# alasdairforsythe/tokenmonster

Measured on AMD Instinct MI355X. Metric: GB/s raw UTF-8 tokenized, englishcode-32000 vocab, higher is better.
Workload: dtype u8; 1 GPU; englishcode-32000-consistent vocabulary shape (synthetic, 32000 ids / 54181 index records), 1024 MiB raw synthetic mixed text per GPU in 300327 documents; end to end: input = RAW UTF-8 resident in HBM, normalized (NFD+capcode) on the GPU inside the timed step, output = uint32 ids + offsets in HBM; raw_bytes_per_gpu=1073743404, normalized_bytes_per_gpu=1145560274, missing=0, parallelism=documents sharded by rank, no collective, rccl_ranks=0

## Files before the change

### tokenmonster_amd/csrc/tm_kernels.hip

```cpp
#include <hip/hip_runtime.h>

#include <algorithm>
#include <chrono>
#include <cstring>
#include <type_traits>
#include <vector>

#include "tm_pipeline.h"

namespace tmh {


__global__ void k_doc_nseg(const uint64_t* __restrict__ doc_begin, const uint64_t* __restrict__ doc_end, uint32_t ndocs,
                           uint32_t* __restrict__ doc_nseg, uint32_t unit = SEG, uint32_t* __restrict__ zero_word = nullptr) {
  uint32_t d = blockIdx.x * blockDim.x + threadIdx.x;
  if (zero_word && d == 0) *zero_word = 0u;
  if (d < ndocs) {
    uint64_t len = doc_end[d] - doc_begin[d];
    doc_nseg[d] = (uint32_t)((len + unit - 1) / unit);
  }
}


__global__ void k_scan_partial(const uint32_t* __restrict__ in, uint64_t n, uint64_t* __restrict__ block_sums) {
// ... 152 lines not shown

template <int FD>
__device__ __forceinline__ uint32_t transition(const Tables& T, const WaveLds& w, const uint8_t* s_bb, int p, int dl,
                                               uint32_t d, const Row& O) {
  if (d == 0) return (T.unk_id != TM_NONE ? T.unk_id : ID_NONE) | (1u << 24) | (1u << 31);
  const int len = (int)desc_len(d);
  const uint32_t id = O.x & kRowIdMask;
  const int i1 = p + len;
  uint32_t res = id | ((uint32_t)len << 24);
  if (i1 < dl && ((O.w & (1u << 21)) == 0 || ((d >> D_NEXT_SPACE) & 1u) == 0u)) {
    const int len1 = (int)(O.w & 63u), len2 = (int)((O.w >> 6) & 63u);
    const int flen[3] = {len, len1 - FD, len2 - FD};
    const int fpart[3] = {len + (int)(O.x >> kRowIdBits) - FD * (100 + (int)((O.w >> 18) & 1u)),
                          (int)(O.y >> kRowIdBits) - FD * (101 + (int)((O.w >> 19) & 1u)),
                          (int)(O.z >> kRowIdBits) - FD * (101 + (int)((O.w >> 20) & 1u))};
    const uint32_t fb[3] = {((O.w >> 12) & 1u) | (((O.w >> 15) & 1u) << 8), ((O.w >> 13) & 1u) | (((O.w >> 16) & 1u) << 8),
                            ((O.w >> 14) & 1u) | (((O.w >> 17) & 1u) << 8)};
    const int nk = len1 == 0 ? 1 : (len2 == 0 ? 2 : 3);
    int best = NOSCORE, bestb = NOSCORE;
    uint32_t resb = 0;
#pragma unroll
    for (int k = 0; k < 3; k++) {
      if (k < nk) {
        const int ik = p + flen[k];
        const uint32_t dS = w.D[ik];
        if (dS != 0) {
          int sc = branch_score(fpart[k], fb[k], dS, false);
          if (k > 0) sc -= alt_penalty(flen[k], dS, len);
          const uint32_t rk = (k == 0 ? id : ((k == 1 ? O.y : O.z) & kRowIdMask)) | ((uint32_t)flen[k] << 24);
          if (sc > best) { best = sc; res = rk; }
          if (dS & D_HAS_B) {
            const uint32_t dB = w.Db[ik];
            int sb = branch_score(fpart[k], fb[k], dB, true);
            if (k > 0) sb -= alt_penalty(flen[k], dB, len);
            if (sb > bestb) { bestb = sb; resb = rk | (1u << 30); }
          }
        }
      }
    }
    if (bestb > best) res = resb;
  }
  return res;
}

#if defined(TM_DEVEL) || defined(TM_PHASE_TIMERS)
#include "../../tools/devel/tm_devel.h"
#else
#define TM_DBG_ON(x) false
#define PH_INIT
#define PH_INC(i)
#define PH_FLUSH
#define PH(i)
#define PH_COUNT(i, n)
#endif


constexpr uint32_t SP_DL_BITS = 21, SP_LEN_SHIFT = 21, SP_LEN_BITS = 9, SP_SAME_DOC = 1u << 30, SP_MORE_TEXT = 1u << 31, SP_DL_MAX = 1u << 20;
static_assert(SP_DL_MAX < (1u << SP_DL_BITS) && SEG < (1 << SP_LEN_BITS) && SP_LEN_SHIFT + SP_LEN_BITS == 30, "the packed word of a segment record");
__global__ void k_seg_fill(const uint64_t* __restrict__ doc_seg_start, uint32_t ndocs, const uint64_t* __restrict__ doc_begin, const uint64_t* __restrict__ doc_end,
                           const uint64_t* __restrict__ doc_vis, const uint64_t* __restrict__ doc_piece_start, const uint64_t* __restrict__ piece_off, uint64_t nseg,
                           uint32_t* __restrict__ seg_doc, uint4* __restrict__ seg_src, const uint64_t* __restrict__ ctl = nullptr) {
  const uint64_t g = (uint64_t)blockIdx.x * blockDim.x + threadIdx.x;
  if (ctl) nseg = ctl[0];
  if (g >= nseg) return;
  uint32_t dl = 0, dh = ndocs;
  while (dh - dl > 1) {
    const uint32_t mid = dl + (dh - dl) / 2;
    if (doc_seg_start[mid] <= g) dl = mid; else dh = mid;
  }
  seg_doc[g] = dl;
  const uint64_t begin = doc_begin[dl] + (g - doc_seg_start[dl]) * SEG;
  const uint64_t rem = doc_end[dl] - begin, remv = doc_vis[dl] - begin;
  const uint32_t look = remv > (uint64_t)SP_DL_MAX ? SP_DL_MAX : (uint32_t)remv;
  const uint32_t seglen = rem < (uint64_t)SEG ? (uint32_t)rem : (uint32_t)SEG;
  const bool same = g + 1 < nseg && doc_seg_start[dl + 1] > g + 1;
  const uint32_t w = look | (seglen << SP_LEN_SHIFT) | (same ? SP_SAME_DOC : 0u) | (remv > (uint64_t)seglen ? SP_MORE_TEXT : 0u);
  if (doc_piece_start == nullptr) { seg_src[g] = make_uint4((uint32_t)begin, (uint32_t)(begin >> 32) & 0xFFu, 0u, w); return; }
  uint64_t lo = doc_piece_start[dl], hi = doc_piece_start[dl + 1];
  while (hi - lo > 1) {
    const uint64_t mid = (lo + hi) >> 1;
    if (piece_off[mid] <= begin) lo = mid; else hi = mid;
  }
  seg_src[g] = make_uint4((uint32_t)lo, (uint32_t)(begin - piece_off[lo]), (uint32_t)(piece_off[lo + 1] - begin), w);
}

constexpr int J_SKIP = NPOS - SEG, J_PLANE = NPOS;
constexpr int TAIL_TASK0 = 64, TAIL_TASKS = (NPOS - TAIL_TASK0) / 3, REDO0 = 160, REDO_WORDS = (NPOS + 31) / 32;
static_assert(REDO0 + REDO_WORDS <= SEG && offsetof(WaveLds, Db) + 4 * 63 + 6 * 256 + 4 <= offsetof(WaveLds, Xb) + 4 * REDO0, "the bitmap lies behind the dump words");
__global__ __launch_bounds__(WAVES * 64, 8) void k_match_branch(Tables T, const uint8_t* __restrict__ text, uint64_t nseg,
                                                                uint32_t* __restrict__ R0, uint2* __restrict__ side,
                                                                uint32_t* __restrict__ R1, uint32_t* __restrict__ exitmap, uint16_t* __restrict__ exit16,
                                                                int narrow, int dbg, const uint8_t* __restrict__ slab, const uint4* __restrict__ par,
                                                                const uint64_t* __restrict__ ctl = nullptr) {
  __shared__ uint8_t s_bb[256];
  __shared__ WaveLds s_wave[WAVES];
  const int lane = threadIdx.x & 63, wvi = __builtin_amdgcn_readfirstlane((int)(threadIdx.x >> 6));
  TM_LDS_OBJECTS(s_bb, s_wave);
  PH_INIT
  const uint64_t g = (uint64_t)blockIdx.x * WAVES + wvi;
  const uint8_t* const bbp = T.begin_byte;
  const uint4 rec = par[g < nseg ? g : nseg - 1];
  if (ctl) nseg = ctl[0];
  TM_HAVE_IN_SGPRS6(rec.x, rec.w, nseg, text, slab, bbp);
  const uint32_t bbw = reinterpret_cast<const uint32_t*>(bbp)[lane];
  if (g >= nseg) return;
  WaveLds& w = s_wave[wvi];
// ... 434 lines not shown
#pragma unroll
    for (int k = 0; k < N0; k++)
      if (pend(ja[k]) && (ja[k] >> JF) >= (uint32_t)SEG) ja[k] = (ja[k] & JCNT) + J1[(ja[k] >> JF) - SEG];
    for (int round = 0; round < 6; round++) {
      bool anyb = false;
#pragma unroll
      for (int k = 0; k < N0; k++) anyb |= pend(ja[k]) && (ja[k] >> (JF + 6)) == (uint32_t)k;
      if (__builtin_amdgcn_ballot_w64(anyb) == 0ull) break;
#pragma unroll
      for (int k = 0; k < N0; k++) {
        const uint32_t b = bperm(ja[k], ja[k]);
        ja[k] = pend(ja[k]) && (ja[k] >> (JF + 6)) == (uint32_t)k ? (ja[k] & JCNT) + b : ja[k];
      }
      PH_INC(13)
    }
#pragma unroll
    for (int k = N0 - 2; k >= 0; k--) {
      uint32_t b = 0u;
#pragma unroll
      for (int j = k + 1; j < N0; j++) {
        const uint32_t bj = bperm(ja[k], ja[j]);
        b = (ja[k] >> (JF + 6)) == (uint32_t)j ? bj : b;
      }
      ja[k] = pend(ja[k]) ? (ja[k] & JCNT) + b : ja[k];
    }
    uint32_t e1 = jb[0];
    if (__builtin_amdgcn_ballot_w64(lane < ENT / 2 && pend(e1)) != 0ull) {
      uint32_t b = 0u;
#pragma unroll
      for (int j = 0; j < N0; j++) {
        const uint32_t bj = bperm(e1, ja[j]);
        b = (e1 >> (JF + 6)) == (uint32_t)j ? bj : b;
      }
      e1 = pend(e1) ? (e1 & JCNT) + b : e1;
    }
    const bool all_wide = (dbg & 32) != 0;
    auto ok_of = [](uint32_t a) { return (a >> 31) != 0 && ((a >> JF) & JNONE) != JNONE; };
    auto e16 = [&](uint32_t a) -> uint32_t { return ok_of(a) ? (((a >> JF) & JNONE) | ((all_wide ? 511u : min(a & JCNT, 511u)) << 7)) : 0xFFFFu; };
    if (lane < ENT / 2) *reinterpret_cast<uint32_t*>(exit16 + g * ENT + 2 * lane) = e16(ja[0]) | (e16(e1) << 16);
    const bool wide = all_wide || (lane < ENT / 2 && ((ok_of(ja[0]) && (ja[0] & JCNT) >= 511u) || (ok_of(e1) && (e1 & JCNT) >= 511u)));
    if (__any(wide) && lane < ENT / 2) {
      exitmap[g * ENT + 2 * lane] = ok_of(ja[0]) ? ((ja[0] >> JF) & JNONE) | ((ja[0] & JCNT) << 8) : R_INVALID;
      exitmap[g * ENT + 2 * lane + 1] = ok_of(e1) ? ((e1 >> JF) & JNONE) | ((e1 & JCNT) << 8) : R_INVALID;
    }
  }
  PH(7)
  PH_FLUSH
}


__global__ void k_resolve(const uint32_t* __restrict__ exitmap, const uint16_t* __restrict__ exit16, const uint64_t* __restrict__ doc_seg_start, uint32_t ndocs,
                          const uint8_t* __restrict__ doc_entry, uint8_t* __restrict__ seg_entry, uint32_t* __restrict__ seg_tokbase,
                          uint32_t* __restrict__ doc_ntok, uint32_t* __restrict__ error_flag, uint32_t long_segs, uint32_t* __restrict__ doc_fd,
                          uint32_t* __restrict__ doc_missing, const uint64_t* __restrict__ ctl = nullptr) {
  uint32_t d = blockIdx.x * blockDim.x + threadIdx.x;
  if (ctl && d < ndocs && ctl[1] == 0) { doc_ntok[d] = 0u; return; }
  if (d >= ndocs) return;
  doc_fd[d] = 0u; doc_missing[d] = 0u;
  uint64_t g0 = doc_seg_start[d], g1 = doc_seg_start[d + 1];
  if (g1 - g0 > long_segs) return;
  uint32_t e = doc_entry ? doc_entry[d] : 0u, ntok = 0;
  for (uint64_t g = g0; g < g1; g++) {
    seg_entry[g] = (uint8_t)e;
    seg_tokbase[g] = ntok;
    const uint32_t x = exit_entry(exit16, exitmap, g * ENT + e);
    if (x == R_INVALID) { atomicOr(error_flag, 1u); break; }
    e = x & 0xFFu;
    ntok += x >> 8;
  }
  doc_ntok[d] = ntok;
}


template <bool LEAF>
__global__ __launch_bounds__(128) void k_group_compose(const uint32_t* __restrict__ exitmap, const uint16_t* __restrict__ exit16, const uint2* __restrict__ gmap_in, const Group* __restrict__ groups,
                                                       uint32_t first_group, uint2* __restrict__ gmap) {
  const uint32_t gi = first_group + blockIdx.x;
  const Group gr = groups[gi];
  const uint32_t e0 = threadIdx.x;
  if (e0 >= ENT) return;
  uint32_t e = e0, ntok = 0;
  bool ok = true;
  for (uint32_t k = 0; k < gr.nchildren; k++) {
    if (LEAF) {
      const uint32_t x = exit_entry(exit16, exitmap, (uint64_t)(gr.first_child + k) * ENT + e);
      if (x == R_INVALID) { ok = false; break; }
      e = x & 0xFFu;
      ntok += x >> 8;
    } else {
      const uint2 x = gmap_in[(uint64_t)(gr.first_child + k) * ENT + e];
      if (x.x == R_INVALID) { ok = false; break; }
      e = x.x;
      ntok += x.y;
    }
  }
  gmap[(uint64_t)gi * ENT + e0] = ok ? make_uint2(e, ntok) : make_uint2(R_INVALID, 0u);
}

__global__ void k_long_top(const uint2* __restrict__ gmap, const LongDoc* __restrict__ longs, uint32_t nlong, const uint8_t* __restrict__ doc_entry,
                           uint8_t* __restrict__ group_entry, uint32_t* __restrict__ group_base, uint32_t* __restrict__ doc_ntok,
                           uint32_t* __restrict__ error_flag) {
  const uint32_t i = blockIdx.x * blockDim.x + threadIdx.x;
  if (i >= nlong) return;
  const LongDoc ld = longs[i];
  uint32_t e = doc_entry ? doc_entry[ld.doc] : 0u, ntok = 0;
  for (uint32_t k = 0; k < ld.ngroups; k++) {
    const uint32_t gi = ld.first_group + k;
    group_entry[gi] = (uint8_t)e;
    group_base[gi] = ntok;
    const uint2 x = gmap[(uint64_t)gi * ENT + e];
    if (x.x == R_INVALID) { atomicOr(error_flag, 1u); break; }
    e = x.x;
    ntok += x.y;
  }
  doc_ntok[ld.doc] = ntok;
}

template <bool LEAF>
__global__ void k_group_expand(const uint32_t* __restrict__ exitmap, const uint16_t* __restrict__ exit16, const uint2* __restrict__ gmap, const Group* __restrict__ groups, uint32_t first_group,
                               uint32_t ngroups, uint8_t* __restrict__ group_entry, uint32_t* __restrict__ group_base,
                               uint8_t* __restrict__ seg_entry, uint32_t* __restrict__ seg_tokbase, uint32_t* __restrict__ error_flag) {
  const uint32_t t = blockIdx.x * blockDim.x + threadIdx.x;
  if (t >= ngroups) return;
// ... 349 lines not shown
            nmiss += w >> 31;
            if (fits) {
              if (NARROW) { if (id != ID_NONE) rowa[E++] = (uint16_t)id; if (fd) rowa[E++] = (uint16_t)delete_id; }
              else { if (id != ID_NONE) row[E++] = id; if (fd) row[E++] = delete_id; }
            } else {
              if (id != ID_NONE) { if (t.base + E < out_cap) TM_STREAM_STORE(&out[t.base + E], id); E++; }
              if (fd) { if (t.base + E < out_cap) TM_STREAM_STORE(&out[t.base + E], delete_id); E++; }
            }
            p += (w >> 24) & 63u;
            hop++;
            gate = p < seglen ? slack0 + (int)p - (int)E - (int)((fd | direct) << 16) : GATE_DEAD;
          }
        }
      } else if (__builtin_amdgcn_ballot_w64(gate >= 0) == 0ull) break;
    }
    if (direct == 0u) staged = E;
    if (nfd | nmiss) {
      const uint32_t doc = seg_doc[g0 + lane];
      if (nfd) atomicAdd(&doc_fd[doc], nfd);
      if (nmiss) atomicAdd(&doc_missing[doc], nmiss);
    }
  }
  __builtin_amdgcn_wave_barrier();
  __builtin_amdgcn_s_waitcnt(0);
#pragma unroll 4
  for (int s = 0; s < nv; s++) {
    const uint32_t n = (uint32_t)__shfl((int)staged, s);
    const uint64_t base = shfl_u64(t.base, s);
    for (uint32_t j = (uint32_t)lane; j < n; j += 64u) if (base + j < out_cap) TM_STREAM_STORE(&out[base + j], NARROW ? (uint32_t)s_a[NARROW ? s : 0][j] : s_tile[NARROW ? 0 : s][j]);
  }
}

template <bool WIDE, bool OUT16 = false>
__global__ __launch_bounds__(64) void k_emit_list(const uint32_t* __restrict__ R0, const uint2* __restrict__ side,
                                                  const uint32_t* __restrict__ R1, const uint4* __restrict__ par, uint64_t nseg,
                                                  uint32_t delete_id, uint64_t out_cap, uint32_t* __restrict__ out,
                                                  uint32_t* __restrict__ error_flag, uint32_t stage_after, const uint32_t* __restrict__ seg_doc,
                                                  uint32_t* __restrict__ doc_fd, uint32_t* __restrict__ doc_missing, uint32_t no_id,
                                                  const uint64_t* __restrict__ ctl = nullptr) {
  alignas(16) __shared__ uint8_t s_m[TSL][TROW_L];
  __shared__ uint32_t s_side[TSL][9];
  __shared__ uint32_t s_n[TSL];
  __shared__ uint64_t s_base[TSL];
  const int lane = threadIdx.x;
  const uint64_t g0 = (uint64_t)blockIdx.x * TSL;
  if (ctl) { nseg = ctl[0]; if (g0 >= nseg) return; }
  const int nv = (int)(nseg - g0 < (uint64_t)TSL ? nseg - g0 : (uint64_t)TSL);
  const TileSeg t = tile_segment(par, g0 + lane, lane < TSL, nseg);
  constexpr uint32_t SLACK = TSLACK_L;
  const uint8_t* rows_g = reinterpret_cast<const uint8_t*>(R0);
  typedef typename std::conditional<WIDE, uint32_t, uint16_t>::type idt;
  typedef typename std::conditional<OUT16, uint16_t, uint32_t>::type outt;
  outt* const outp = reinterpret_cast<outt*>(out);
  constexpr uint64_t RS = WIDE ? R0_WIDE : R0_NARROW, FO = WIDE ? 4 * SEG : 2 * SEG;
  {
    uint32_t vb[TSL];
#pragma unroll
    for (int s = 0; s < TSL; s++) {
      const int ss = s < nv ? s : nv - 1;
      const uint32_t len = s < nv ? (uint32_t)__shfl((int)t.seglen, ss) : 0u;
      vb[s] = 0u;
      if (4u * (uint32_t)lane < len) vb[s] = TM_STREAM_LOAD(reinterpret_cast<const uint32_t*>(rows_g + (g0 + (uint64_t)ss) * RS + FO) + lane);
    }
#pragma unroll
    for (int s = 0; s < TSL; s++) *reinterpret_cast<uint32_t*>(&s_m[s][TSLACK_L + 4 * lane]) = vb[s];
#pragma unroll
    for (int i = lane; i < TSL * 9; i += 64) reinterpret_cast<uint32_t*>(s_side)[i] = 0u;
    static_assert((TSL & (TSL - 1)) == 0 && TSL >= 8 && TSL <= 64, "a lane per segment, lane & (TSL - 1); the second phase takes eight at a time");
    __builtin_amdgcn_wave_barrier();
    __builtin_amdgcn_s_waitcnt(0);
  }
  uint32_t staged = 0;
  {
    const int rl = lane & (TSL - 1);
    uint8_t* rowm = s_m[rl];
    uint32_t* smap = s_side[rl];
    const uint2* __restrict__ sl = side + (g0 + rl) * SIDE_STRIDE;
    const idt* __restrict__ ids_g = reinterpret_cast<const idt*>(rows_g + (g0 + (uint64_t)(rl < nv ? rl : 0)) * RS);
    uint32_t nfd = 0, nmiss = 0;
    auto word = [&](uint32_t pp, uint32_t f) -> uint32_t {
      if (f != 0) return side_word(sl, R1, g0 + rl, pp);
      const uint32_t m8 = rowm[SLACK + pp];
      return ((m8 >> 7) ? no_id : (uint32_t)ids_g[pp]) | ((m8 & 63u) << 24) | ((m8 >> 6) << 30);
    };
    const uint32_t seglen = t.have ? t.seglen : 0u;
    uint32_t p = t.entry >> 1, fd = t.entry & 1u, E = 0, direct = 0, hop = 0;
    constexpr int GATE_DEAD = -(1 << 24);
    const int slack0 = (int)SLACK - 2 - (int)stage_after;
    int gate = p < seglen ? slack0 + (int)p - (int)(fd << 16) : GATE_DEAD;
    const uint32_t nounk = no_id == ID_NONE ? 1u : 0u;
    auto fast_step = [&]() __attribute__((always_inline)) {
      const uint32_t m8 = rowm[SLACK + p];
      const uint32_t miss = m8 >> 7, fdn = (m8 >> 6) & 1u, adv = m8 & 63u;
      const uint32_t has = 1u - (miss & nounk);
      rowm[E] = (uint8_t)p; E += has; rowm[E] = (uint8_t)p;
      E += fdn;
      gate += (int)adv - (int)(fdn * 0x10001u + has);
      nfd += fdn;
      nmiss += miss;
      fd = fdn;
      p += max(adv, 1u);
      gate = p < seglen ? gate : GATE_DEAD;
    };
    for (;;) {
#ifndef TM_EMU
      if (gate >= 0) {
        do fast_step(); while (__builtin_amdgcn_ballot_w64(gate < 0) == 0ull);
      }
#else
      if (__builtin_amdgcn_ballot_w64(gate >= 0) != 0ull) {
        const bool in = gate >= 0;
        do { if (in) fast_step(); } while (__builtin_amdgcn_ballot_w64(in && gate < 0) == 0ull);
      }
#endif
      const bool general = (uint32_t)gate > (uint32_t)GATE_DEAD;
      if (__builtin_amdgcn_ballot_w64(general) != 0ull) {
        if (general) {
          const uint32_t w = word(p, fd);
          if (w == R_INVALID || hop > 2u * SEG) { atomicOr(error_flag, 2u); p = seglen; gate = GATE_DEAD; }
          else {
            const uint32_t id = w & ID_NONE, adv = (w >> 24) & 63u, fdn = (w >> 30) & 1u;
            const bool fits = direct == 0u && slack0 + (int)p - (int)E >= 0 && adv != 0u && !(id == ID_NONE && fdn != 0u);
            if (!fits && direct == 0u) { direct = 1u; staged = E; }
            nfd += fdn;
            nmiss += w >> 31;
            if (fits) {
              if (id != ID_NONE) {
                if (fd) { smap[E >> 5] |= 1u << (E & 31u); if (t.base + E < out_cap) TM_STREAM_STORE(&outp[t.base + E], (outt)id); }
                rowm[E++] = (uint8_t)p;
              }
              if (fdn) rowm[E++] = (uint8_t)p;
            } else {
              if (id != ID_NONE) { if (t.base + E < out_cap) TM_STREAM_STORE(&outp[t.base + E], (outt)id); E++; }
              if (fdn) { if (t.base + E < out_cap) TM_STREAM_STORE(&outp[t.base + E], (outt)delete_id); E++; }
            }
            fd = fdn;
            p += adv;
            hop++;
            gate = p < seglen ? slack0 + (int)p - (int)E - (int)((fd | direct) << 16) : GATE_DEAD;
          }
        }
      } else if (__builtin_amdgcn_ballot_w64(gate >= 0) == 0ull) break;
    }
    if (direct == 0u) staged = E;
    if (nfd | nmiss) {
      const uint32_t doc = seg_doc[g0 + lane];
      if (nfd) atomicAdd(&doc_fd[doc], nfd);
      if (nmiss) atomicAdd(&doc_missing[doc], nmiss);
    }
  }
  __builtin_amdgcn_wave_barrier();
  __builtin_amdgcn_s_waitcnt(0);
  if (out_cap == 0) return;
  if (lane < TSL) { s_n[lane] = lane < nv ? staged : 0u; s_base[lane] = t.base; }
  __builtin_amdgcn_wave_barrier();
  __builtin_amdgcn_s_waitcnt(0);
  uint32_t nmax = 0;
#pragma unroll
  for (int s = 0; s < TSL; s++) nmax = max(nmax, s_n[s]);
  nmax = (uint32_t)__builtin_amdgcn_readfirstlane((int)nmax);
  for (uint32_t j0 = 0; j0 < nmax; j0 += 64u) {
    const uint32_t j = j0 + (uint32_t)lane, jj = min(j, (uint32_t)TROW_L - 1u), jp = max(jj, 1u) - 1u;
#pragma unroll 1
    for (int s0 = 0; s0 < TSL; s0 += 8) {
      uint32_t idv[8];
#pragma unroll
      for (int k = 0; k < 8; k++) {
        const int s = s0 + k, ss = s < nv ? s : nv - 1;
        const uint32_t pp = s_m[s][jj], prev = s_m[s][jp];
        const uint32_t fetched = reinterpret_cast<const idt*>(rows_g + (g0 + (uint64_t)ss) * RS)[pp];
        idv[k] = (pp == prev && j != 0u) ? delete_id : fetched;
      }
#pragma unroll
      for (int k = 0; k < 8; k++) {
        const int s = s0 + k;
        const uint64_t base = s_base[s];
        const bool written = ((s_side[s][jj >> 5] >> (jj & 31u)) & 1u) != 0u;
        if (j < s_n[s] && !written && base + j < out_cap) TM_STREAM_STORE(&outp[base + j], (outt)idv[k]);
      }
    }
  }
}

template <int WV>
__global__ __launch_bounds__(WV * 64) void k_score_tiles(const uint32_t* __restrict__ R0, const uint2* __restrict__ side,
                                                        const uint32_t* __restrict__ R1, const uint8_t* __restrict__ text,
                                                        const uint4* __restrict__ par, uint64_t nseg, uint32_t delete_id,
                                                        uint32_t* __restrict__ scores, unsigned long long* __restrict__ tokens,
                                                        uint32_t* __restrict__ missing_bits, uint32_t* __restrict__ error_flag, int narrow, uint32_t no_id) {
  alignas(16) __shared__ uint32_t s_tile[WV][TS][TROW];
  alignas(16) __shared__ unsigned long long s_w[HSLOTS];
  __shared__ unsigned long long s_ntok;
  __shared__ uint32_t s_ndel;
  for (int j = threadIdx.x; j < HSLOTS; j += WV * 64) s_w[j] = HEMPTY;
  if (threadIdx.x == 0) { s_ntok = 0; s_ndel = 0; }
  __syncthreads();
  const int lane = threadIdx.x & 63, wv = __builtin_amdgcn_readfirstlane((int)(threadIdx.x >> 6));
  uint32_t ntok = 0, ndel = 0;
  for (uint64_t g0 = ((uint64_t)blockIdx.x * WV + wv) * TS; g0 < nseg; g0 += (uint64_t)gridDim.x * WV * TS) {
    const int nv = (int)(nseg - g0 < (uint64_t)TS ? nseg - g0 : (uint64_t)TS);
    const TileSeg t = tile_segment(par, g0 + lane, lane < TS, nseg);
    tile_load(s_tile[wv], t, g0, nv, lane, R0, narrow, no_id);
    uint32_t staged = 0;
    {
      const int rl = lane & (TS - 1);
      uint32_t* row = s_tile[wv][rl];
      const uint32_t seglen = t.have ? t.seglen : 0u;
      uint32_t p = t.entry >> 1, fd = t.entry & 1u, hop = 0;
      const uint2* __restrict__ sl = side + (g0 + rl) * SIDE_STRIDE;
      for (;;) {
        const bool alive = p < seglen;
        if (!__any(alive)) break;
        const bool slow = alive && (fd != 0u || staged >= TSLACK + p);
        if (__any(slow)) {
          if (slow) {
            const uint32_t w = fd != 0u ? side_word(sl, R1, g0 + rl, p) : row[TSLACK + p];
            if (w == R_INVALID || hop > 2u * SEG) { atomicOr(error_flag, 2u); p = seglen; }
            else {
              fd = (w >> 30) & 1u;
              if (w >> 31) {
                const uint32_t byte = text[t.begin + p];
                atomicOr(&missing_bits[byte >> 5], 1u << (byte & 31));
              } else if (staged < TSLACK + p) row[staged++] = w;
              else atomicAdd(&scores[w & ID_NONE], (w >> 24) & 63u);
              ntok += 1 + fd;
              ndel += fd;
              p += (w >> 24) & 63u;
              hop++;
            }
          }
        }
        if (alive && !slow) {
          const uint32_t w = row[TSLACK + p];
          if (w == R_INVALID) atomicOr(error_flag, 2u);
// ... 498 lines not shown
    for (uint32_t g = b->level_first[lvl]; g < b->level_first[lvl + 1]; g++) groups[g].first_child += b->level_first[lvl - 1];
  for (size_t i = 0; i < longs.size(); i++) longs[i].first_group = b->level_first[tops[i].level] + tops[i].first;
  b->ngroups = (uint32_t)groups.size();
  b->nlong = (uint32_t)longs.size();
  if (b->ngroups == 0) return TM_OK;
  hipError_t e;
  { int rc = reserve_groups(b, b->ngroups, b->nlong); if (rc != TM_OK) return rc; }
  const size_t gb = groups.size() * sizeof(Group), lb = longs.size() * sizeof(LongDoc), lat = (gb + 255) & ~(size_t)255;
  std::memcpy(b->h_groups, groups.data(), gb);
  std::memcpy(b->h_groups + lat, longs.data(), lb);
  if ((e = hipMemcpyAsync(b->d_groups, b->h_groups, gb, hipMemcpyHostToDevice, st)) != hipSuccess ||
      (e = hipMemcpyAsync(b->d_longs, b->h_groups + lat, lb, hipMemcpyHostToDevice, st)) != hipSuccess ||
      (e = hipStreamSynchronize(st)) != hipSuccess)
    return hip_fail(e, "H2D segment groups");
  return TM_OK;
}

int pipeline_match(tm_batch* b, hipStream_t st, hipEvent_t* ev, bool for_score) {
  const tm_vocab* v = b->vocab;
  { int rc = enter_device(v); if (rc != TM_OK) return rc; }
  b->last_stream = st;
  (void)hipGetLastError();
  auto mark = [&](int k) { if (ev) (void)hipEventRecord(ev[k], st); };
  const uint32_t nd = b->ndocs;
  const uint64_t nseg = b->nseg;
  if (nd == 0) (void)hipMemsetAsync(b->d_error, 0, 4, st);
  mark(0);
  if (nd > 0) {
    TM_LAUNCH(k_doc_nseg, (nd + 255) / 256, 256, 0, st, b->d_doc_begin, b->d_doc_end, nd, b->d_doc_nseg, (uint32_t)SEG, b->d_error);
    scan_u32(b->d_doc_nseg, nd, b->d_scan_tmp, b->d_totals + 0, b->d_doc_seg_start, st);
    if (nseg > 0)
      TM_LAUNCH(k_seg_fill, (uint32_t)((nseg + 255) / 256), 256, 0, st, b->d_doc_seg_start, nd, b->d_doc_begin, b->d_doc_end, b->d_doc_vis ? b->d_doc_vis : b->d_doc_end,
                b->text_in_slabs ? b->d_doc_piece_start : nullptr, b->d_piece_off, nseg, b->d_seg_doc, b->d_seg_par, b->d_ctl);
  }
  mark(1);
  if (nseg > 0)
    TM_LAUNCH(k_match_branch, (uint32_t)((nseg + WAVES - 1) / WAVES), WAVES * 64, TM_K1_EXTRA_LDS, st, v->tables, b->d_text, nseg, b->d_R0, b->d_side, b->d_R1, b->d_exitmap,
              b->d_exit16, r0_mode(b, for_score), debug_flags(), b->text_in_slabs ? b->d_slab : nullptr, b->d_seg_par, b->d_ctl);
    note_table_use(v, st);
  mark(2);
  for (size_t lvl = 0; lvl + 1 < b->level_first.size() && b->ngroups > 0; lvl++) {
    const uint32_t g0 = b->level_first[lvl], ng = b->level_first[lvl + 1] - g0;
    if (lvl == 0) TM_LAUNCH(k_group_compose<true>, ng, 128, 0, st, b->d_exitmap, b->d_exit16, b->d_gmap, b->d_groups, g0, b->d_gmap);
    else TM_LAUNCH(k_group_compose<false>, ng, 128, 0, st, b->d_exitmap, b->d_exit16, b->d_gmap, b->d_groups, g0, b->d_gmap);
  }
  hipError_t e = hipGetLastError();
  return e == hipSuccess ? TM_OK : hip_fail(e, "kernel launch");
}

int pipeline_resolve(tm_batch* b, hipStream_t st, hipEvent_t* ev, int mode) {
  (void)hipGetLastError();
  const uint32_t nd = b->ndocs;
  auto mark = [&](int k) { if (ev) (void)hipEventRecord(ev[k], st); };
  if (nd > 0)
    TM_LAUNCH(k_resolve, (nd + 255) / 256, 256, 0, st, b->d_exitmap, b->d_exit16, b->d_doc_seg_start, nd, b->d_doc_entry, b->d_seg_entry, b->d_seg_tokbase,
                                                b->d_doc_ntok, b->d_error, long_segs(), b->d_doc_fd, b->d_doc_missing, b->d_ctl);
  if (b->ngroups > 0) {
    TM_LAUNCH(k_long_top, (b->nlong + 63) / 64, 64, 0, st, b->d_gmap, b->d_longs, b->nlong, b->d_doc_entry, b->d_group_entry, b->d_group_base, b->d_doc_ntok, b->d_error);
    for (size_t lvl = b->level_first.size() - 1; lvl-- > 0;) {
      const uint32_t g0 = b->level_first[lvl], ng = b->level_first[lvl + 1] - g0;
      if (lvl == 0) TM_LAUNCH(k_group_expand<true>, (ng + 63) / 64, 64, 0, st, b->d_exitmap, b->d_exit16, b->d_gmap, b->d_groups, g0, ng, b->d_group_entry, b->d_group_base,
                                                                         b->d_seg_entry, b->d_seg_tokbase, b->d_error);
      else TM_LAUNCH(k_group_expand<false>, (ng + 63) / 64, 64, 0, st, b->d_exitmap, b->d_exit16, b->d_gmap, b->d_groups, g0, ng, b->d_group_entry, b->d_group_base,
                                                                 b->d_seg_entry, b->d_seg_tokbase, b->d_error);
    }
  }
  mark(3);
  if (nd > 0) scan_u32(b->d_doc_ntok, nd, b->d_scan_tmp, b->d_totals + 1, b->d_tok_offsets, st);
  else (void)hipMemsetAsync(b->d_tok_offsets, 0, 8, st);
  mark(4);
  if (mode > 0) launch_emit(b, st, mode == 2);
  mark(5);
  hipError_t e = hipGetLastError();
  return e == hipSuccess ? TM_OK : hip_fail(e, "kernel launch");
}

void launch_doc_exits(tm_batch* b, uint8_t* d_exits, hipStream_t st) {
  if (b->ndocs) TM_LAUNCH(k_doc_exits, b->ndocs, 128, 0, st, b->d_exitmap, b->d_exit16, b->d_doc_seg_start, b->d_gmap, b->d_longs, b->nlong, d_exits, long_segs());
}

void launch_enc_carry(tm_batch* b, const uint8_t* d_exits, uint8_t* d_entry, uint32_t* d_acc, uint64_t own, uint32_t keep, hipStream_t st) {
  TM_LAUNCH(k_enc_carry, 1, 256, 0, st, d_exits, d_entry, b->d_doc_missing, d_acc, b->d_text, own, keep);
}

int run_pipeline(tm_batch* b, hipStream_t st, bool timed, float* ms, bool emit) {
  hipError_t e;
  if (timed && !b->have_events) {
    for (auto& ev : b->ev) if ((e = hipEventCreate(&ev)) != hipSuccess) return hip_fail(e, "hipEventCreate");
    b->have_events = true;
  }
  b->has_output = false;
  b->row_form = -1;
  int rc = pipeline_match(b, st, timed ? b->ev : nullptr);
  if (rc == TM_OK) rc = pipeline_resolve(b, st, timed ? b->ev : nullptr, emit ? 2 : 1);
  if (rc != TM_OK) return rc;
  b->has_output = emit;
  if (emit) b->row_form = r0_mode(b, false);
  if (timed) {
    if ((e = hipEventSynchronize(b->ev[TM_NUM_KERNELS])) != hipSuccess) return hip_fail(e, "hipEventSynchronize");
    for (int k = 0; k < TM_NUM_KERNELS; k++) (void)hipEventElapsedTime(&ms[k], b->ev[k], b->ev[k + 1]);
  }
  return TM_OK;
}

__global__ void k_copy_small(const uint8_t* __restrict__ src, uint8_t* __restrict__ dst, uint64_t n, int words) {
  const uint64_t i = (uint64_t)blockIdx.x * blockDim.x + threadIdx.x;
  if (words) { if (i < n / 8) reinterpret_cast<uint64_t*>(dst)[i] = reinterpret_cast<const uint64_t*>(src)[i]; }
  else if (i < n) dst[i] = src[i];
}
// ... 138 lines not shown
    hipStream_t st = b->last_stream;
    launch_emit(b, st, true, true);
    if ((e = hipStreamSynchronize(st)) != hipSuccess) return hip_fail(e, "emit rerun");
  }
  return TM_OK;
}

}

extern "C" {

const char* tm_kernel_name(int k) { return k >= 0 && k < TM_NUM_KERNELS ? kKernelNames[k] : ""; }

int tm_debug_flags(int flags) {
  const int old = tmh::debug_flags();
  if (flags >= 0 && tmh::hooks_armed()) tmh::g_debug_flags = flags & tmh::kDebugMask;
  return old;
}

}
namespace tmh {
int make_workspace(const tm_vocab* v, uint64_t max_bytes, uint32_t max_docs, bool own_text, bool with_output, tm_batch** out) {
  *out = nullptr;
  { int rc = enter_device(v); if (rc != TM_OK) return rc; }
  auto* b = new tm_batch();
  b->vocab = v;
  b->max_bytes = max_bytes;
  b->max_docs = max_docs;
  b->max_segs = max_bytes / SEG + max_docs + 1;
  b->out_cap = with_output ? max_bytes / 2 + 2ull * max_docs + 1024 : 0;
  b->text_borrowed = !own_text;
  const uint64_t nd1 = (uint64_t)max_docs + 1;
  const uint64_t scan_blocks = (nd1 + max_bytes / 256 + 2 * SCAN_CH) / SCAN_CH + 64;
  hipError_t e = hipSuccess;
  if ((own_text && (e = dalloc(b, &b->d_text, max_bytes + 256)) != hipSuccess) || (e = dalloc(b, &b->d_offsets, 2 * nd1)) != hipSuccess ||
      (e = dalloc(b, &b->d_doc_nseg, nd1)) != hipSuccess || (e = dalloc(b, &b->d_doc_seg_start, nd1 + 1)) != hipSuccess ||
      (e = dalloc(b, &b->d_seg_doc, b->max_segs)) != hipSuccess || (e = dalloc(b, &b->d_R0, b->max_segs * (v->host.n_ids <= 65536u ? SEG : SEG + SEG / 4))) != hipSuccess || (e = dalloc(b, &b->d_R1, b->max_segs * SEG)) != hipSuccess ||
      (e = dalloc(b, &b->d_side, b->max_segs * SIDE_STRIDE)) != hipSuccess ||
      (e = dalloc(b, &b->d_exitmap, b->max_segs * ENT)) != hipSuccess || (e = dalloc(b, &b->d_exit16, b->max_segs * ENT)) != hipSuccess || (e = dalloc(b, &b->d_seg_entry, b->max_segs)) != hipSuccess ||
      (e = dalloc(b, &b->d_seg_tokbase, b->max_segs)) != hipSuccess || (e = dalloc(b, &b->d_seg_par, b->max_segs + 1)) != hipSuccess || (e = dalloc(b, &b->d_doc_ntok, nd1)) != hipSuccess ||
      (e = dalloc(b, &b->d_doc_events, nd1)) != hipSuccess || (e = dalloc(b, &b->d_doc_missing, nd1)) != hipSuccess || (e = dalloc(b, &b->d_doc_fd, nd1)) != hipSuccess ||
      (e = dalloc(b, &b->d_tok_offsets, nd1 + 1)) != hipSuccess || (e = dalloc(b, &b->d_scan_tmp, scan_blocks)) != hipSuccess ||
      (e = dalloc(b, &b->d_totals, 8)) != hipSuccess ||
      (e = dalloc(b, &b->d_out, b->out_cap)) != hipSuccess) {
    tm_batch_free(b);
    return hip_fail(e, "hipMalloc (batch workspace)");
  }
  {
    const uint64_t nlong_max = b->max_segs / LONG_SEGS + 1, ngroups_max = b->max_segs / GROUP_FAN + b->max_segs / (GROUP_FAN * GROUP_FAN) + 3 * nlong_max + 64;
    int rc = reserve_groups(b, (uint32_t)std::min<uint64_t>(ngroups_max, 1u << 30), (uint32_t)std::min<uint64_t>(nlong_max, 1u << 30));
    if (rc != TM_OK) { tm_batch_free(b); return rc; }
  }
  (void)hipMemset(b->d_totals, 0, 64);
  b->d_error = reinterpret_cast<uint32_t*>(b->d_totals + 4);
  *out = b;
  return TM_OK;
}
int make_piece_workspace(const tm_vocab* v, uint64_t max_bytes, hipStream_t st, tm_batch** out) {
  *out = nullptr;
  { int rc = enter_device(v); if (rc != TM_OK) return rc; }
  auto* b = new tm_batch();
  b->vocab = v;
  b->max_bytes = max_bytes;
  b->max_docs = 1;
  b->max_segs = max_bytes / SEG + 2;
  const uint64_t scan_blocks = (2 + max_bytes / 256 + 2 * SCAN_CH) / SCAN_CH + 64;
  hipError_t e = hipSuccess;
  if ((e = dalloc(b, &b->d_text, max_bytes + 256)) != hipSuccess || (e = dalloc(b, &b->d_scan_tmp, scan_blocks)) != hipSuccess || (e = dalloc(b, &b->d_totals, 8)) != hipSuccess ||
      (e = hipMemsetAsync(b->d_totals, 0, 64, st)) != hipSuccess) {
    tm_batch_free(b);
    return hip_fail(e, "hipMalloc (piece workspace)");
  }
  b->d_error = reinterpret_cast<uint32_t*>(b->d_totals + 4);
  *out = b;
  return TM_OK;
}
}
extern "C" {

int tm_batch_create(const tm_vocab* v, uint64_t max_bytes, uint32_t max_docs, tm_batch** out) {
  if (!v || !out) return set_error(TM_E_INVALID, "null argument");
  return make_workspace(v, max_bytes, max_docs, true, true, out);
}

void tm_batch_free(tm_batch* b) {
  if (!b) return;
  void* ptrs[] = {b->text_borrowed ? nullptr : (void*)b->d_text, b->d_offsets, b->d_doc_nseg, b->d_doc_seg_start, b->d_seg_doc, b->d_R0, b->d_R1, b->d_side, b->d_exitmap, b->d_exit16, b->d_seg_entry,
                  b->d_seg_tokbase, b->d_seg_par, b->d_doc_ntok, b->d_doc_events, b->d_doc_missing, b->d_doc_fd, b->d_tok_offsets, b->d_scan_tmp, b->d_totals,
                  b->d_out, b->d_groups, b->d_longs, b->d_gmap, b->d_group_entry, b->d_group_base,
                  b->d_ctl_store, b->d_dec_a, b->d_dec_b, b->d_spans, b->d_own, b->d_own_tmp, b->d_win, b->d_win_rows, b->d_units[0], b->d_units[1]};
  for (void* p : ptrs) (void)hipFree(p);
  tmh::raw_free(b);
  if (b->have_events) for (auto& ev : b->ev) (void)hipEventDestroy(ev);
  if (b->aux_stream) (void)hipStreamDestroy(b->aux_stream);
  (void)hipHostFree(b->h_fb_raw); (void)hipHostFree(b->h_fb_norm); (void)hipHostFree(b->h_mail); (void)hipHostFree(b->h_groups);
  delete b;
}

int tm_batch_upload(tm_batch* b, const uint8_t* text, const uint64_t* offsets, uint32_t ndocs) {
  int rc = tmh::batch_upload_on(b, text, offsets, ndocs, nullptr);
  if (rc == TM_OK) { hipError_t e = hipStreamSynchronize(nullptr); if (e != hipSuccess) rc = hip_fail(e, "H2D text"); }
  return rc;
}

}
namespace tmh {
// ... 157 lines not shown
```

### tokenmonster_amd/csrc/tm_pipeline.h

```cpp
#pragma once
#include <hip/hip_runtime.h>

#include <cstdint>
#include <mutex>
#include <vector>

#include "tm_device.h"
#include "tm_norm_masks.h"

namespace tmh {

constexpr int SEG = 256;
constexpr int NPOS = SEG + 40;
constexpr int NPOS_PAD = (NPOS + 63) / 64 * 64;
constexpr int TEXT_LEN = SEG + 96;
constexpr int RAW_PIECE = 1024;
constexpr int SLAB_BYTES = 2048;
constexpr int ENT = 80;
#ifndef TM_K1_WAVES
#define TM_K1_WAVES 4
#endif
constexpr int WAVES = TM_K1_WAVES;
constexpr uint32_t R_INVALID = 0xFFFFFFFFu;
constexpr uint32_t J_EXIT = 1024;
constexpr uint32_t J_INVALID = 2047;
constexpr uint32_t ID_NONE = 0xFFFFFFu;
constexpr int NOSCORE = -1000000;
constexpr int SIDE_STRIDE = 16;
constexpr uint32_t SIDE_DENSE = 0xFFFFFFFFu;
constexpr uint32_t LONG_SEGS = 512;

constexpr int SCAN_T = 256, SCAN_PER = 16, SCAN_CH = SCAN_T * SCAN_PER;

constexpr uint32_t GROUP_FAN = 64;
struct Group { uint32_t first_child, nchildren, doc, level; };
struct LongDoc { uint32_t doc, first_group, ngroups, pad; };

__device__ __forceinline__ uint32_t sel_mask(unsigned long long mask, uint32_t a, uint32_t b) {
#ifdef TM_EMU
  return ((mask >> emu::cur->lane) & 1ull) ? a : b;
#else
  uint32_t r;
  asm("v_cndmask_b32_e64 %0, %1, %2, %3" : "=v"(r) : "v"(b), "v"(a), "s"(mask));
  return r;
#endif
}
__device__ __forceinline__ uint32_t bit_of(uint32_t x, uint32_t n) {
#ifdef TM_EMU
  return (x >> (n & 31u)) & 1u;
#else
  return __builtin_amdgcn_ubfe(x, n, 1u);
#endif
}
__device__ __forceinline__ uint32_t add_mask_bit(uint32_t a, unsigned long long mask) {
#ifdef TM_EMU
  return a + (uint32_t)((mask >> emu::cur->lane) & 1ull);
#else
  uint32_t r;
  unsigned long long carry_out;
  asm("v_addc_co_u32_e64 %0, %1, %2, 0, %3" : "=v"(r), "=s"(carry_out) : "v"(a), "s"(mask));
  return r;
#endif
}
__device__ __forceinline__ uint32_t read_lane(uint32_t v, int l) {
#ifdef TM_EMU
  return __shfl(v, l);
#else
  return (uint32_t)__builtin_amdgcn_readlane((int)v, l);
#endif
}
#ifdef TM_EMU
static inline uint32_t tm_dpp_emu(uint32_t old, uint32_t src, int ctrl, int rows) {
  const int lane = (int)emu::cur->lane, row = lane >> 4;
  int from = lane; bool have = false;
  if (ctrl > 0x110 && ctrl <= 0x11F) { from = lane - (ctrl - 0x110); have = (lane & 15) >= ctrl - 0x110; }
  else if (ctrl == 0x138) { from = lane - 1; have = lane >= 1; }
  else if (ctrl == 0x130) { from = lane + 1; have = lane < 63; }
  else if (ctrl == 0x142) { from = row * 16 - 1; have = row >= 1; }
  else if (ctrl == 0x143) { from = 31; have = row >= 2; }
  const uint32_t v = __shfl(src, from & 63);
  return (have && ((rows >> row) & 1)) ? v : old;
}
#define TM_DPP(old, src, ctrl, rows) tm_dpp_emu(old, src, ctrl, rows)
// ... 27 lines not shown
#define TM_K4_TSL 16
#endif
constexpr int TSL = TM_K4_TSL, TSLACK_L = 4, TROW_L = SEG + 16;

struct TileSeg { bool have; uint64_t begin, base; uint32_t seglen, entry; };
__device__ __forceinline__ TileSeg tile_segment(const uint4* __restrict__ par, uint64_t g, bool lane_ok, uint64_t nseg) {
  TileSeg t{lane_ok && g < nseg, 0, 0, 0, 0};
  if (t.have) {
    const uint4 q = par[g];
    t.begin = (uint64_t)q.x | ((uint64_t)(q.y & 0xFFu) << 32);
    t.seglen = (q.y >> 8) & 0xFFFu;
    t.entry = (q.y >> 20) & 0x7Fu;
    t.base = (uint64_t)q.z | ((uint64_t)q.w << 32);
  }
  return t;
}
__device__ __forceinline__ uint32_t side_word(const uint2* __restrict__ sl, const uint32_t* __restrict__ R1, uint64_t g, uint32_t p) {
  const uint32_t nside = sl[0].x;
  if (nside == SIDE_DENSE) return R1[g * SEG + p];
  uint32_t w = R_INVALID;
  for (uint32_t k = 1; k <= nside && k < (uint32_t)SIDE_STRIDE; k++) { const uint2 sv = sl[k]; if (sv.x == p) w = sv.y; }
  return w;
}

}

struct tm_batch {
  const tm_vocab* vocab = nullptr;
  uint64_t max_bytes = 0;
  uint32_t max_docs = 0;
  uint64_t max_segs = 0;
  uint64_t nbytes = 0, nseg = 0;
  uint32_t ndocs = 0;
  uint64_t device_bytes = 0;
  hipStream_t last_stream = nullptr;
  hipStream_t aux_stream = nullptr;
  uint8_t* d_text = nullptr;
  bool text_borrowed = false;
  uint64_t* d_offsets = nullptr;
  const uint64_t* d_doc_begin = nullptr;
  const uint64_t* d_doc_end = nullptr;
  const uint64_t* d_doc_vis = nullptr;
  const uint8_t* d_doc_entry = nullptr;
  uint32_t* d_doc_nseg = nullptr;
  uint64_t* d_doc_seg_start = nullptr;
  uint32_t* d_seg_doc = nullptr;
  uint32_t* d_R0 = nullptr;
  uint2* d_side = nullptr;
  uint32_t* d_R1 = nullptr;
  uint32_t* d_exitmap = nullptr;
  uint16_t* d_exit16 = nullptr;
  uint8_t* d_seg_entry = nullptr;
  uint32_t* d_seg_tokbase = nullptr;
  uint4* d_seg_par = nullptr;
  uint32_t* d_doc_ntok = nullptr;
  uint32_t* d_doc_events = nullptr;
  uint32_t* d_doc_missing = nullptr;
  uint32_t* d_doc_fd = nullptr;
  uint64_t* d_tok_offsets = nullptr;
  uint64_t* d_scan_tmp = nullptr;
  uint64_t* d_totals = nullptr;
  uint32_t* d_error = nullptr;
  uint32_t ngroups = 0, nlong = 0, cap_groups = 0, cap_long = 0;
  std::vector<uint32_t> level_first;
  tmh::Group* d_groups = nullptr;
  tmh::LongDoc* d_longs = nullptr;
  uint2* d_gmap = nullptr;
  uint8_t* d_group_entry = nullptr;
  uint32_t* d_group_base = nullptr;
  uint8_t* d_raw = nullptr;
  uint8_t* d_rawf = nullptr; uint64_t rawf_cap = 0;
  uint64_t* d_rawf_off = nullptr; uint64_t rawf_docs_cap = 0;
  uint8_t* d_pf_piece = nullptr; uint64_t pf_piece_cap = 0;
  void* d_pf_doc = nullptr;
  uint32_t* d_acc = nullptr;
  uint8_t* d_slab = nullptr;
  uint64_t slab_pieces = 0;
  bool text_in_slabs = false;
  uint64_t slab_cap = 0;
  uint64_t* d_raw_off = nullptr;
  uint64_t raw_cap = 0, raw_bytes = 0, raw_pieces = 0, piece_cap = 0;
  uint32_t raw_docs = 0, raw_docs_cap = 0;
  std::vector<uint64_t> h_raw_off;
  uint32_t host_fallback_docs = 0;
  uint32_t* d_doc_npiece = nullptr;
  uint64_t* d_doc_piece_start = nullptr;
  uint32_t* d_piece_doc = nullptr;
  uint32_t* d_piece_sum = nullptr;
  uint8_t* d_piece_carry = nullptr;
  uint32_t* d_piece_len = nullptr;
  uint64_t* d_piece_off = nullptr;
  tmh::NmTwo* d_two = nullptr;
  uint8_t* d_need_host = nullptr;
  uint64_t* d_nbegin = nullptr;
  uint64_t* d_nend = nullptr;
  uint64_t* d_ninfo = nullptr;
  uint64_t* d_fb_roff = nullptr; uint64_t* d_fb_noff = nullptr; uint32_t* d_fb_ids = nullptr;
  uint8_t* h_mail = nullptr; uint64_t mail_pos = 0;
  uint8_t* h_groups = nullptr; uint64_t h_groups_cap = 0;
  struct MailPending { void* dst; const uint8_t* slot; uint64_t n; hipStream_t st; };
  std::vector<MailPending> mail_pending;
  std::vector<hipStream_t> mail_streams;
  uint64_t last_totals[3] = {0, 0, 0};
  uint8_t* h_fb_raw = nullptr; uint8_t* h_fb_norm = nullptr;
  uint64_t h_fb_raw_cap = 0, h_fb_norm_cap = 0;
  uint32_t* d_out = nullptr;
// ... 165 lines not shown
```

Measured before the change: 48.44 GB/s.

## Resolve mid-length documents with a wave per document instead of one thread

k_resolve now hands documents with more than RESOLVE_WAVE_MIN segments (but fewer than the long-doc threshold) to a new k_resolve_wave kernel through a device-side work list kept in the seg_par buffer. That kernel stages blocks of 64 segments' exit maps into LDS with coalesced 16-byte loads, prefetches the next block, and walks the entry chain from LDS, writing seg_entry and tokbase for 64 lanes at once. The goal is to remove the slow serial per-thread walk over scattered global exit16 entries for mid-length documents. In exchange it adds a kernel launch, atomics on a counter, reuse of the seg_par scratch buffer, and entry clamping to 127. It also adds phase-timer macro hooks that compile to nothing by default.

Result: no change. 48.48 GB/s, median of 2 (+0.1%).

```diff
diff --git a/tokenmonster_amd/csrc/tm_kernels.hip b/tokenmonster_amd/csrc/tm_kernels.hip
--- a/tokenmonster_amd/csrc/tm_kernels.hip
+++ b/tokenmonster_amd/csrc/tm_kernels.hip
@@ -228,6 +228,8 @@
 #define PH_FLUSH
 #define PH(i)
 #define PH_COUNT(i, n)
+#define PH4_INIT
+#define PH4_FLUSH
 #endif
 
 
@@ -768,13 +770,14 @@
 __global__ void k_resolve(const uint32_t* __restrict__ exitmap, const uint16_t* __restrict__ exit16, const uint64_t* __restrict__ doc_seg_start, uint32_t ndocs,
                           const uint8_t* __restrict__ doc_entry, uint8_t* __restrict__ seg_entry, uint32_t* __restrict__ seg_tokbase,
                           uint32_t* __restrict__ doc_ntok, uint32_t* __restrict__ error_flag, uint32_t long_segs, uint32_t* __restrict__ doc_fd,
-                          uint32_t* __restrict__ doc_missing, const uint64_t* __restrict__ ctl = nullptr) {
+                          uint32_t* __restrict__ doc_missing, uint32_t* __restrict__ wave_count, uint32_t* __restrict__ wave_docs, const uint64_t* __restrict__ ctl = nullptr) {
   uint32_t d = blockIdx.x * blockDim.x + threadIdx.x;
   if (ctl && d < ndocs && ctl[1] == 0) { doc_ntok[d] = 0u; return; }
   if (d >= ndocs) return;
   doc_fd[d] = 0u; doc_missing[d] = 0u;
   uint64_t g0 = doc_seg_start[d], g1 = doc_seg_start[d + 1];
   if (g1 - g0 > long_segs) return;
+  if (g1 - g0 > RESOLVE_WAVE_MIN) { wave_docs[atomicAdd(&wave_count[0], 1u)] = d; return; }
   uint32_t e = doc_entry ? doc_entry[d] : 0u, ntok = 0;
   for (uint64_t g = g0; g < g1; g++) {
     seg_entry[g] = (uint8_t)e;
@@ -785,6 +788,69 @@
     ntok += x >> 8;
   }
   doc_ntok[d] = ntok;
+}
+
+constexpr int RW_SEGS = 64;
+constexpr int RW_Q = RW_SEGS * ENT * 2 / 16 / 64;
+constexpr uint32_t RW_ENTRY_MAX = 127;
+__global__ __launch_bounds__(64) void k_resolve_wave(const uint32_t* __restrict__ exitmap, const uint16_t* __restrict__ exit16, const uint64_t* __restrict__ doc_seg_start,
+                                                     const uint8_t* __restrict__ doc_entry, uint8_t* __restrict__ seg_entry, uint32_t* __restrict__ seg_tokbase,
+                                                     uint32_t* __restrict__ doc_ntok, uint32_t* __restrict__ error_flag, uint32_t* __restrict__ wave_count, const uint32_t* __restrict__ wave_docs) {
+  static_assert(RW_Q * 16 * 64 == RW_SEGS * ENT * 2 && (ENT * 2) % 16 == 0, "a block's maps are whole 16-byte loads of the 64 lanes");
+  alignas(16) __shared__ uint16_t s_map[RW_SEGS * ENT + RW_ENTRY_MAX + 1 - ENT];
+  const int lane = threadIdx.x;
+  const uint32_t n = __atomic_load_n(&wave_count[0], __ATOMIC_RELAXED);
+  uint32_t mine = 0;
+  for (uint32_t i = blockIdx.x; i < n; i += gridDim.x, mine++) {
+    const uint32_t d = wave_docs[i];
+    const uint64_t g0 = doc_seg_start[d], g1 = doc_seg_start[d + 1];
+    uint32_t e = doc_entry ? min((uint32_t)doc_entry[d], RW_ENTRY_MAX) : 0u, ntok = 0;
+    uint4 q[RW_Q];
+    auto fetch = [&](uint64_t g) __attribute__((always_inline)) {
+      const uint32_t nq = (uint32_t)(g1 - g < (uint64_t)RW_SEGS ? g1 - g : (uint64_t)RW_SEGS) * (uint32_t)(ENT * 2 / 16);
+      const uint4* __restrict__ src = reinterpret_cast<const uint4*>(exit16 + g * ENT);
+#pragma unroll
+      for (int k = 0; k < RW_Q; k++) {
+        const uint32_t at = (uint32_t)lane + 64u * (uint32_t)k;
+        q[k] = at < nq ? src[at] : make_uint4(0u, 0u, 0u, 0u);
+      }
+    };
+    fetch(g0);
+    bool ok = true;
+    for (uint64_t g = g0; g < g1 && ok; g += RW_SEGS) {
+      __syncthreads();
+#pragma unroll
+      for (int k = 0; k < RW_Q; k++) reinterpret_cast<uint4*>(s_map)[lane + 64 * k] = q[k];
+      __syncthreads();
+      if (g + RW_SEGS < g1) fetch(g + RW_SEGS);
+      const uint32_t nb = (uint32_t)__builtin_amdgcn_readfirstlane((int)(g1 - g < (uint64_t)RW_SEGS ? g1 - g : (uint64_t)RW_SEGS));
+      uint32_t my_e = 0, my_base = 0, nw = nb, ntok_bad = 0;
+      for (uint32_t k0 = 0; k0 < nb; k0 += 8u) {
+        const uint16_t* maps = s_map + k0 * ENT;
+#pragma unroll
+        for (uint32_t j = 0; j < 8u; j++) {
+          const uint32_t k = k0 + j;
+          my_e = (uint32_t)lane == k ? e : my_e;
+          my_base = (uint32_t)lane == k ? ntok : my_base;
+          const uint32_t x16 = maps[j * ENT + e];
+          uint32_t c = x16 >> 7, en = x16 & 0x7Fu;
+          if (__builtin_amdgcn_ballot_w64(c == 511u) != 0ull) {
+            const uint32_t x = x16 == 0xFFFFu ? R_INVALID : exitmap[(g + k) * ENT + e];
+            if (x == R_INVALID && ok) { if (lane == 0) atomicOr(error_flag, 1u); ok = false; nw = k + 1u; ntok_bad = ntok; }
+            en = x == R_INVALID ? 0u : min(x & 0xFFu, RW_ENTRY_MAX);
+            c = x == R_INVALID ? 0u : x >> 8;
+          }
+          e = en;
+          ntok += c;
+        }
+      }
+      if (!ok) ntok = ntok_bad;
+      else if ((nb & 7u) != 0u) { e = (uint32_t)__shfl((int)my_e, (int)nb); ntok = (uint32_t)__shfl((int)my_base, (int)nb); }
+      if ((uint32_t)lane < nw) { seg_entry[g + lane] = (uint8_t)my_e; seg_tokbase[g + lane] = my_base; }
+    }
+    if (lane == 0) doc_ntok[d] = ntok;
+  }
+  if (lane == 0 && mine != 0u && atomicAdd(&wave_count[1], mine) + mine == n) { atomicExch(&wave_count[1], 0u); atomicExch(&wave_count[0], 0u); }
 }
 
 
@@ -1240,6 +1306,7 @@
   typedef typename std::conditional<WIDE, uint32_t, uint16_t>::type idt;
   typedef typename std::conditional<OUT16, uint16_t, uint32_t>::type outt;
   outt* const outp = reinterpret_cast<outt*>(out);
+  PH4_INIT
   constexpr uint64_t RS = WIDE ? R0_WIDE : R0_NARROW, FO = WIDE ? 4 * SEG : 2 * SEG;
   {
     uint32_t vb[TSL];
@@ -1258,6 +1325,7 @@
     __builtin_amdgcn_wave_barrier();
     __builtin_amdgcn_s_waitcnt(0);
   }
+  PH(0)
   uint32_t staged = 0;
   {
     const int rl = lane & (TSL - 1);
@@ -1339,7 +1407,8 @@
   }
   __builtin_amdgcn_wave_barrier();
   __builtin_amdgcn_s_waitcnt(0);
-  if (out_cap == 0) return;
+  PH(1)
+  if (out_cap == 0) { PH4_FLUSH return; }
   if (lane < TSL) { s_n[lane] = lane < nv ? staged : 0u; s_base[lane] = t.base; }
   __builtin_amdgcn_wave_barrier();
   __builtin_amdgcn_s_waitcnt(0);
@@ -1359,6 +1428,7 @@
         const uint32_t fetched = reinterpret_cast<const idt*>(rows_g + (g0 + (uint64_t)ss) * RS)[pp];
         idv[k] = (pp == prev && j != 0u) ? delete_id : fetched;
       }
+      PH(2)
 #pragma unroll
       for (int k = 0; k < 8; k++) {
         const int s = s0 + k;
@@ -1366,8 +1436,10 @@
         const bool written = ((s_side[s][jj >> 5] >> (jj & 31u)) & 1u) != 0u;
         if (j < s_n[s] && !written && base + j < out_cap) TM_STREAM_STORE(&outp[base + j], (outt)idv[k]);
       }
-    }
-  }
+      PH(3)
+    }
+  }
+  PH4_FLUSH
 }
 
 template <int WV>
@@ -1972,9 +2044,14 @@
   (void)hipGetLastError();
   const uint32_t nd = b->ndocs;
   auto mark = [&](int k) { if (ev) (void)hipEventRecord(ev[k], st); };
-  if (nd > 0)
+  if (nd > 0) {
     TM_LAUNCH(k_resolve, (nd + 255) / 256, 256, 0, st, b->d_exitmap, b->d_exit16, b->d_doc_seg_start, nd, b->d_doc_entry, b->d_seg_entry, b->d_seg_tokbase,
-                                                b->d_doc_ntok, b->d_error, long_segs(), b->d_doc_fd, b->d_doc_missing, b->d_ctl);
+                                                b->d_doc_ntok, b->d_error, long_segs(), b->d_doc_fd, b->d_doc_missing, b->d_wave_count, reinterpret_cast<uint32_t*>(b->d_seg_par), b->d_ctl);
+    const uint64_t listed_max = b->nseg / (RESOLVE_WAVE_MIN + 1);
+    if (listed_max > 0)
+      TM_LAUNCH(k_resolve_wave, (uint32_t)std::min<uint64_t>(listed_max, RESOLVE_WAVE_GRID), 64, 0, st, b->d_exitmap, b->d_exit16, b->d_doc_seg_start, b->d_doc_entry, b->d_seg_entry,
+                                                b->d_seg_tokbase, b->d_doc_ntok, b->d_error, b->d_wave_count, reinterpret_cast<const uint32_t*>(b->d_seg_par));
+  }
   if (b->ngroups > 0) {
     TM_LAUNCH(k_long_top, (b->nlong + 63) / 64, 64, 0, st, b->d_gmap, b->d_longs, b->nlong, b->d_doc_entry, b->d_group_entry, b->d_group_base, b->d_doc_ntok, b->d_error);
     for (size_t lvl = b->level_first.size() - 1; lvl-- > 0;) {
@@ -2219,6 +2296,7 @@
     if (rc != TM_OK) { tm_batch_free(b); return rc; }
   }
   (void)hipMemset(b->d_totals, 0, 64);
+  b->d_wave_count = reinterpret_cast<uint32_t*>(b->d_totals + 6);
   b->d_error = reinterpret_cast<uint32_t*>(b->d_totals + 4);
   *out = b;
   return TM_OK;
diff --git a/tokenmonster_amd/csrc/tm_pipeline.h b/tokenmonster_amd/csrc/tm_pipeline.h
--- a/tokenmonster_amd/csrc/tm_pipeline.h
+++ b/tokenmonster_amd/csrc/tm_pipeline.h
@@ -29,6 +29,11 @@
 constexpr int SIDE_STRIDE = 16;
 constexpr uint32_t SIDE_DENSE = 0xFFFFFFFFu;
 constexpr uint32_t LONG_SEGS = 512;
+#ifndef TM_RESOLVE_WAVE_MIN
+#define TM_RESOLVE_WAVE_MIN 64
+#endif
+constexpr uint32_t RESOLVE_WAVE_MIN = TM_RESOLVE_WAVE_MIN;
+constexpr uint64_t RESOLVE_WAVE_GRID = 4096;
 
 constexpr int SCAN_T = 256, SCAN_PER = 16, SCAN_CH = SCAN_T * SCAN_PER;
 
@@ -162,6 +167,7 @@
   uint16_t* d_exit16 = nullptr;
   uint8_t* d_seg_entry = nullptr;
   uint32_t* d_seg_tokbase = nullptr;
+  uint32_t* d_wave_count = nullptr;
   uint4* d_seg_par = nullptr;
   uint32_t* d_doc_ntok = nullptr;
   uint32_t* d_doc_events = nullptr;
```
